# tnestmeyer/reflectance-filtering

Hardware: AMD Instinct MI355X
Metric: megapixels/sec joint-bilateral sigma_c=20 sigma_s=22 @1080p (higher is better)
Workload: dtype f32

## Files before the change

include/reflectance_filtering.h:

```cpp
#ifndef REFLECTANCE_FILTERING_H
#define REFLECTANCE_FILTERING_H

#include <stddef.h>
#include <stdint.h>

#ifdef __cplusplus
extern "C" {
#endif

#define RF_VERSION 103

#define RF_OK 0
#define RF_E_BADARG (-1)
#define RF_E_UNSUPPORTED (-2)
#define RF_E_WORKSPACE (-3)
#define RF_E_HIP (-4)

#define RF_BORDER_CONSTANT 0
#define RF_BORDER_REPLICATE 1
#define RF_BORDER_REFLECT 2
#define RF_BORDER_WRAP 3
#define RF_BORDER_REFLECT_101 4
#define RF_BORDER_DEFAULT RF_BORDER_REFLECT_101

#define RF_JBF_TRUE_DIVISION 1
#define RF_JBF_FORCE_GENERIC 2
#define RF_JBF_GREY_AS_BGR 4

int rf_version(void);
const char *rf_last_error(void);
int rf_shutdown(void);

int rf_jbf_u8(const uint8_t *joint, const uint8_t *src, uint8_t *dst, int n, int h, int w,
              int joint_cn, int src_cn, int d, double sigma_color, double sigma_space, int border,
              int flags, void *stream);

size_t rf_jbf_ragged_workspace_bytes(int n, const int *heights, const int *widths, int joint_cn,
                                     int src_cn, int d, double sigma_space, int flags);
int rf_jbf_ragged_u8(const uint8_t *joint, const uint8_t *src, uint8_t *dst, int n,
                     const int *heights, const int *widths, int joint_cn, int src_cn, int d,
                     double sigma_color, double sigma_space, int border, int flags, void *workspace,
                     size_t workspace_bytes, void *stream);

size_t rf_gf_workspace_bytes(int n, int h, int w, int guide_cn, int src_cn, int radius);
int rf_gf_u8(const uint8_t *guide, const uint8_t *src, uint8_t *dst, int n, int h, int w,
             int guide_cn, int src_cn, int radius, double eps, int iterations, void *workspace,
// ... 104 lines not shown
```

include/reflectance_filtering_debug.h:

```cpp
#ifndef REFLECTANCE_FILTERING_DEBUG_H
#define REFLECTANCE_FILTERING_DEBUG_H

#ifdef __cplusplus
extern "C" {
#endif

int rf_debug_option(const char *name, int value);

int rf_debug_clock_probe(unsigned long long *out2, int micros, void *stream);

const char *rf_debug_build_info(void);

int rf_debug_jbf_points_plan(int n_params, const double *sigma_space, int d, int joint_cn, int flags,
                             int total_points, int *out, int max_chunks);

int rf_debug_jbf_ragged_plan(int n, const int *heights, const int *widths, int joint_cn, int src_cn,
                             int d, double sigma_color, double sigma_space, int flags, int *out,
                             int cap);

int rf_debug_jbf_ragged_slab_plan(int n, const int *heights, const int *widths, int joint_cn,
                                  int src_cn, int d, double sigma_color, double sigma_space, int flags,
                                  int *out, int cap);

int rf_debug_colorize_ragged_plan(int n, const int *heights, const int *widths, int *out, int cap);

int rf_debug_gf_ragged_plan(int n, const int *heights, const int *widths, int guide_cn, int src_cn,
                            int radius, int flags, int *out, int cap);

int rf_debug_png_plan(int n, const int *heights, const int *widths, int cn_in, int flags, int *out,
                      int cap);

#ifdef __cplusplus
}
#endif
#endif
```

reflectance_filtering_amd/_ffi.py:

```python
import ctypes
import os
import threading

_HERE = os.path.dirname(os.path.abspath(__file__))
LIB_PATH = os.path.join(_HERE, "librf_hip.so")

RF_OK, RF_E_BADARG, RF_E_UNSUPPORTED, RF_E_WORKSPACE, RF_E_HIP = 0, -1, -2, -3, -4
BORDER_CONSTANT, BORDER_REPLICATE, BORDER_REFLECT, BORDER_WRAP, BORDER_REFLECT_101 = range(5)
BORDER_DEFAULT = BORDER_REFLECT_101
JBF_TRUE_DIVISION = 1
JBF_FORCE_GENERIC = 2
JBF_GREY_AS_BGR = 4
GF_GREY_AS_BGR = 1
PNG_GREY_AS_RGB = 1
PNG_FLAG_GREY, PNG_FLAG_BAD_FILTER = 1, 2
CNN_NPARAMS = 4513
CNN_NPACKED = 4673
CNN_NCHW_RGB, CNN_NHWC_BGR = 0, 1
CNN_LAYOUTS = {"nchw_rgb": CNN_NCHW_RGB, "nhwc_bgr": CNN_NHWC_BGR}

EXPORTS = ("rf_version", "rf_last_error", "rf_shutdown", "rf_jbf_u8", "rf_gf_workspace_bytes",
           "rf_gf_u8", "rf_gf_ex_u8", "rf_cnn_reflectance_u8", "rf_cnn_pack_weights",
           "rf_cnn_reflectance_packed_u8", "rf_colorize_workspace_bytes",
           "rf_colorize_srgb_u8", "rf_whdr_f32", "rf_jbf_f32_workspace_bytes", "rf_jbf_f32",
           "rf_gf_f32_workspace_bytes", "rf_gf_f32", "rf_jbf_points_workspace_bytes",
           "rf_jbf_points_u8", "rf_jbf_points_ragged_workspace_bytes", "rf_jbf_points_ragged_u8",
           "rf_whdr_points_u8", "rf_jbf_ragged_workspace_bytes", "rf_jbf_ragged_u8",
           "rf_colorize_ragged_workspace_bytes", "rf_colorize_ragged_srgb_u8",
           "rf_gf_ragged_workspace_bytes", "rf_gf_ragged_u8", "rf_png_stream_bound",
           "rf_png_workspace_bytes", "rf_png_deflate_ragged_u8",
           "rf_png_unfilter_workspace_bytes", "rf_png_unfilter_ragged_u8",
           "rf_colorize_ragged_r8_srgb_u8", "rf_cnn_reflectance_f32",
           "rf_cnn_reflectance_packed_f32")

DEBUG_EXPORTS = ("rf_debug_option", "rf_debug_clock_probe", "rf_debug_build_info",
                 "rf_debug_jbf_points_plan", "rf_debug_jbf_ragged_plan",
                 "rf_debug_jbf_ragged_slab_plan", "rf_debug_colorize_ragged_plan",
                 "rf_debug_gf_ragged_plan", "rf_debug_png_plan")
RESULT_CHANGING_OPTIONS = ("jbf_stage_only", "gf_exp_skip")

_lib = None
_lock = threading.Lock()


class RFError(RuntimeError):
    """A librf_hip.so entry point returned a negative code."""


def load_library():
    global _lib
    with _lock:
        if _lib is not None:
            return _lib
        import torch
        if not os.path.exists(LIB_PATH):
            raise RFError("%s not found: build it with `python -c 'import __graft_entry__ as g; "
                          "g.build()'` or `make -C reflectance_filtering_amd/csrc` "
                          "(there is no CPU fallback)" % LIB_PATH)
        lib = ctypes.CDLL(LIB_PATH)
        vp, ci, cd, sz = ctypes.c_void_p, ctypes.c_int, ctypes.c_double, ctypes.c_size_t
        lib.rf_version.argtypes = []
        lib.rf_version.restype = ci
        lib.rf_last_error.argtypes = []
        lib.rf_last_error.restype = ctypes.c_char_p
        lib.rf_shutdown.argtypes = []
        lib.rf_shutdown.restype = ci
        lib.rf_jbf_u8.argtypes = [vp, vp, vp, ci, ci, ci, ci, ci, ci, cd, cd, ci, ci, vp]
        lib.rf_jbf_u8.restype = ci
        lib.rf_gf_workspace_bytes.argtypes = [ci, ci, ci, ci, ci, ci]
        lib.rf_gf_workspace_bytes.restype = sz
        lib.rf_gf_u8.argtypes = [vp, vp, vp, ci, ci, ci, ci, ci, ci, cd, ci, vp, sz, vp]
        lib.rf_gf_u8.restype = ci
        lib.rf_gf_ex_u8.argtypes = [vp, vp, vp, ci, ci, ci, ci, ci, ci, cd, ci, ci, vp, sz, vp]
        lib.rf_gf_ex_u8.restype = ci
        lib.rf_gf_ragged_workspace_bytes.argtypes = [ci, vp, vp, ci, ci, ci, ci]
        lib.rf_gf_ragged_workspace_bytes.restype = sz
        lib.rf_gf_ragged_u8.argtypes = [vp, vp, vp, ci, vp, vp, ci, ci, ci, cd, ci, ci, vp, sz, vp]
        lib.rf_gf_ragged_u8.restype = ci
        lib.rf_cnn_reflectance_u8.argtypes = [vp, vp, vp, ci, ci, ci, vp, vp, vp]
        lib.rf_cnn_reflectance_u8.restype = ci
        lib.rf_cnn_pack_weights.argtypes = [vp, vp, vp]
# ... 55 lines not shown
        lib.rf_png_unfilter_ragged_u8.restype = ci
        lib.rf_debug_png_plan.argtypes = [ci, vp, vp, ci, ci, vp, ci]
        lib.rf_debug_png_plan.restype = ci
        lib.rf_debug_option.argtypes = [ctypes.c_char_p, ci]
        lib.rf_debug_option.restype = ci
        lib.rf_debug_clock_probe.argtypes = [vp, ci, vp]
        lib.rf_debug_clock_probe.restype = ci
        lib.rf_debug_build_info.argtypes = []
        lib.rf_debug_build_info.restype = ctypes.c_char_p
        lib.rf_debug_jbf_points_plan.argtypes = [ci, vp, ci, ci, ci, ci, vp, ci]
        lib.rf_debug_jbf_points_plan.restype = ci
        lib.rf_debug_jbf_ragged_plan.argtypes = [ci, vp, vp, ci, ci, ci, cd, cd, ci, vp, ci]
        lib.rf_debug_jbf_ragged_plan.restype = ci
        lib.rf_debug_jbf_ragged_slab_plan.argtypes = [ci, vp, vp, ci, ci, ci, cd, cd, ci, vp, ci]
        lib.rf_debug_jbf_ragged_slab_plan.restype = ci
        lib.rf_debug_colorize_ragged_plan.argtypes = [ci, vp, vp, vp, ci]
        lib.rf_debug_colorize_ragged_plan.restype = ci
        lib.rf_debug_gf_ragged_plan.argtypes = [ci, vp, vp, ci, ci, ci, ci, vp, ci]
        lib.rf_debug_gf_ragged_plan.restype = ci
        import sys
        for item in filter(None, os.environ.get("RF_DEBUG_OPTIONS", "").split(",")):
            name, _, value = item.partition("=")
            name = name.strip()
            try:
                number = int(value or 1)
            except ValueError:
                raise RFError("RF_DEBUG_OPTIONS: %r is not an integer (option %r)" % (value, name))
            if lib.rf_debug_option(name.encode(), number) < 0:
                raise RFError("RF_DEBUG_OPTIONS: unknown debug option %r" % name)
            if name in RESULT_CHANGING_OPTIONS and number:
# ... 82 lines not shown
    hs = np.ascontiguousarray(sizes[:, 0], dtype=np.int32)
    ws = np.ascontiguousarray(sizes[:, 1], dtype=np.int32)
    out = np.zeros(7, dtype=np.int32)
    args = (sizes.shape[0], hs.ctypes.data, ws.ctypes.data, int(joint_cn), int(src_cn), int(d),
            float(sigma_color), float(sigma_space), int(flags), out.ctypes.data, 1)
    rc = lib.rf_debug_jbf_ragged_slab_plan(*args)
    if rc == -1:
        if sizes.shape[0] == 0 or lib.rf_jbf_ragged_workspace_bytes(*(args[:6] + (args[7], args[8]))) > 0:
            return None
        lib.rf_debug_jbf_ragged_slab_plan(*args)
    if rc < 0:
        check(rc, "rf_debug_jbf_ragged_slab_plan")
    return tuple(int(v) for v in out)


def colorize_ragged_plan(sizes):
    import numpy as np
    lib = load_library()
    sizes = np.asarray(sizes, dtype=np.int64).reshape(-1, 2)
    n = sizes.shape[0]
    hs = np.ascontiguousarray(sizes[:, 0], dtype=np.int32)
    ws = np.ascontiguousarray(sizes[:, 1], dtype=np.int32)
    out = np.zeros(n + 2, dtype=np.int32)
    rc = lib.rf_debug_colorize_ragged_plan(n, hs.ctypes.data, ws.ctypes.data, out.ctypes.data, n + 2)
    if rc < 0:
        check(rc, "rf_debug_colorize_ragged_plan")
    return int(out[0]), int(out[1]), [int(v) for v in out[2:]]


def gf_ragged_plan(sizes, guide_cn, src_cn, radius, flags=0):
# ... 42 lines not shown
```

reflectance_filtering_amd/csrc/rf_api.hip:

```cpp
#include "rf_common.hpp"

#include <atomic>
#include <cstring>

#include "reflectance_filtering_debug.h"

namespace rf {

void jbf_shutdown();
void cnn_shutdown();
void gf_shutdown();

char *last_error_buf()
{
    static thread_local char buf[512] = "";
    return buf;
}

int fail(int code, const char *fmt, ...)
{
    va_list ap;
    va_start(ap, fmt);
    vsnprintf(last_error_buf(), 512, fmt, ap);
    va_end(ap);
// ... 6 lines not shown

}

extern "C" int rf_debug_option(const char *name, int value)
{
    static const char *const names[] = {"gf_two_kernel",     "jbf_stage_only",
                                                      "jbf_compiler_loop", "jbf_tile64_only",
                                                      "jbf_tune",          "jbf_f32_untiled",
                                                      "cnn_lds_columns",   "gf_seg_rows",
                                                      "gf_one_stream",     "gf_force_two_streams",
                                                      "gf_guide_cache",    "gf_chained",        "gf_no_compact",
                                                      "gf_exp_skip",       "gf_stagger",        "gf_parts",
                                                      "gf_s1_cap",         "gf_s1_min_wgs",
                                                      "jbf_lookahead1",    "gf_s1_legacy_strips",
                                                      "gf_exact_all_flagged", "gf_cw_chan_run",   "gf_exact",
                                                      "jbf_no_msad",       "colorize_chunk_px"};
    static_assert(sizeof(names) / sizeof(names[0]) == rf::kDbgCount, "one name per DebugOption");
    if (name)
        for (int i = 0; i < rf::kDbgCount; i++)
            if (std::strcmp(name, names[i]) == 0)
                return rf::g_debug[i].exchange(value < 0 ? 0 : value);
    return rf::fail(RF_E_BADARG, "rf_debug_option: unknown option '%s'", name ? name : "(null)");
}

__global__ void clock_probe_kernel(unsigned long long *out, unsigned long long ticks)
{
    if (threadIdx.x != 0)
        return;
    const unsigned long long r0 = __builtin_amdgcn_s_memrealtime();
    const unsigned long long c0 = __builtin_amdgcn_s_memtime();
    unsigned long long r1 = r0;
// ... 21 lines not shown
extern "C" int rf_version(void) { return RF_VERSION | 0x40000000; }
#else
extern "C" int rf_version(void) { return RF_VERSION; }
#endif

#ifndef RF_TOOLCHAIN
#define RF_TOOLCHAIN "unknown toolchain"
#endif
extern "C" const char *rf_debug_build_info(void) { return RF_TOOLCHAIN; }

extern "C" const char *rf_last_error(void) { return rf::last_error_buf(); }

extern "C" int rf_shutdown(void)
{
    rf::jbf_shutdown();
    rf::cnn_shutdown();
    rf::gf_shutdown();
    return RF_OK;
}
```

reflectance_filtering_amd/csrc/rf_common.hpp:

```cpp
#pragma once
#include <hip/hip_runtime.h>

#include <cstdarg>
#include <cstdint>
#include <cstdio>

#include "reflectance_filtering.h"

namespace rf {

char *last_error_buf();
int fail(int code, const char *fmt, ...);

#define RF_HIP_CHECK(expr)                                                                   \
    do {                                                                                     \
        hipError_t _e = (expr);                                                              \
        if (_e != hipSuccess)                                                                \
            return ::rf::fail(RF_E_HIP, "%s failed: %s (%s:%d)", #expr, hipGetErrorString(_e), \
                              __FILE__, __LINE__);                                           \
    } while (0)

__host__ __device__ inline int border_interpolate(int p, int len, int border)
{
    if ((unsigned)p < (unsigned)len)
// ... 60 lines not shown
    kDbgGfGuideCache,
    kDbgGfChained,
    kDbgGfNoCompact,
    kDbgGfExpSkip,
    kDbgGfStagger,
    kDbgGfParts,
    kDbgGfS1Cap,
    kDbgGfS1MinWgs,
    kDbgJbfLookahead1,
    kDbgGfS1LegacyStrips,
    kDbgGfExactAllFlagged,
    kDbgGfCwChanRun,
    kDbgGfExact,
    kDbgJbfNoMsad,
    kDbgColorizeChunkPx,
    kDbgCount
};
int debug_get(int id);

}
```

reflectance_filtering_amd/csrc/rf_jbf.hip:

```cpp
#include <algorithm>
#include <mutex>
#include <vector>

#include "rf_jbf_common.hpp"
#include "rf_jbf_tables.hpp"
#include "rf_jbf_taploops.hpp"

namespace rf {
namespace {

constexpr int kTileW = 64;
constexpr int kMaxLds = 160 * 1024;
constexpr int kTlw2 = 144;
constexpr int kJbfMaxTiledR4 = 468;
constexpr int kJbfStageOnly = 0x1000, kJbfCompilerLoop = 0x2000, kJbfTile64Only = 0x4000;
constexpr int kJbfLookahead1 = 0x8000;
constexpr int kJbfNoMsad = 0x10000;

int jbf_debug_flags()
{
    return (debug_get(kDbgJbfStageOnly) ? kJbfStageOnly : 0) |
           (debug_get(kDbgJbfCompilerLoop) ? kJbfCompilerLoop : 0) |
           (debug_get(kDbgJbfTile64Only) ? kJbfTile64Only : 0) |
           (debug_get(kDbgJbfLookahead1) ? kJbfLookahead1 : 0) |
           (debug_get(kDbgJbfNoMsad) ? kJbfNoMsad : 0);
}

__device__ inline void load_packed4(const uint8_t *img, size_t pix, int cn, uint32_t (&out)[4])
{
    const uint8_t *p = img + pix * (cn < 0 ? 1 : cn);
    if (cn == 3) {
        uint32_t d0, d1, d2;
// ... 242 lines not shown
struct alignas(16) JbfTileRec {
    unsigned long long first;
    int h, w, tile_y0, tile_x0, pad[2];
};
static_assert(sizeof(JbfTileRec) == 32, "the workspace holds 32 bytes per tile");

template <bool kRagged>
struct JbfTilesArg {
    using type = int;
};
template <>
struct JbfTilesArg<true> {
    using type = const JbfTileRec *__restrict__;
};

template <int SCN, int GREP, int CREP, int TLW, int TH = 64, bool kRagged = false>
__global__ __launch_bounds__(1024) void jbf_tile64_kernel(
    const uint8_t *__restrict__ joint, const uint8_t *__restrict__ src, uint8_t *__restrict__ dst,
    int h, int w, int jcn, int radius, int border, const float *__restrict__ lut, int nz,
    const int *__restrict__ hwtab, const float *__restrict__ swsym, int sw_len,
    typename JbfTilesArg<kRagged>::type tiles_x, int tiles_per_img, int flags, int crows, int y_base,
    int x_base)
{
    constexpr int NT = 1024;
    constexpr int QW = NT / TH;
    constexpr int TW = 4 * QW;
    static_assert(TH == 64 || TH == 32 || ((TH == 16 || TH == 128) && SCN == 1), "tile shapes");
    static_assert(QW >= 32 || (QW == 16 && TLW % 32 == 16) || (QW == 8 && TLW % 32 == 8),
                  "row pitch keeps the rows of a half-wave on disjoint banks");
    constexpr int Q4 = TLW / 4;
    extern __shared__ __align__(16) unsigned char smem[];
    volatile int *flag_word = reinterpret_cast<volatile int *>(smem);
    const bool need_sw = (flags & (kJbfCompilerLoop | kJbfLookahead1)) != 0;
    float *swl = reinterpret_cast<float *>(smem + 16);
    const int sw_bytes = need_sw ? ((radius + 1) * sw_len * 4 + 15) & ~15 : 0;
    unsigned char *tile_raw = smem + 16 + sw_bytes;
    if (threadIdx.x == 0)
        *flag_word = 3;
// ... 232 lines not shown
        w[i] = 0xdeadbeefu;
    __syncthreads();
    uint32_t bad = 0;
    const uint32_t addrs[4] = {(uint32_t)kT64Lds + 4u * threadIdx.x, (uint32_t)kT64Lds + 61056u,
                               262140u, (uint32_t)kT64Lds - 4u};
#pragma unroll
    for (int k = 0; k < 4; k++) {
        uint32_t v;
        asm volatile("ds_read_b32 %0, %1\n s_waitcnt lgkmcnt(0)" : "=v"(v) : "v"(addrs[k]));
        bad |= (k < 3) ? (v != 0u) : (v != 0xdeadbeefu);
    }
    if (bad)
        atomicOr(out, 1u);
}

struct Tiled2Config {
    int th, lutrep;
    bool full_lut;
};

size_t tiled2_lds_bytes(const JbfTables &t, int th, int lutrep, bool full_lut)
{
    const int lut_len = full_lut ? 256 * t.joint_cn : t.lut_len;
    const size_t lut_bytes = ((size_t)lut_len * lutrep * 4 + 15) & ~(size_t)15;
    const size_t sw_bytes = ((size_t)(t.radius + 1) * t.sw_len * 4 + 15) & ~(size_t)15;
    return 16 + lut_bytes + sw_bytes + (size_t)kTlw2 * (th + 2 * t.radius) * sizeof(uint2);
}

template <int SCN, int TH, int LUTREP>
int launch_tiled2(const JbfTables &t, bool full_lut, const uint8_t *joint, const uint8_t *src,
// ... 9 lines not shown
        return fail(RF_E_UNSUPPORTED, "rf_jbf_u8: batch too large for one launch");
    auto kern = clamp ? jbf_tiled2_kernel<SCN, TH, LUTREP, true>
                      : jbf_tiled2_kernel<SCN, TH, LUTREP, false>;
    RF_HIP_CHECK(hipFuncSetAttribute((const void *)kern, hipFuncAttributeMaxDynamicSharedMemorySize,
                                     (int)lds));
    hipLaunchKernelGGL(kern, dim3((unsigned)blocks), dim3(16 * TH), lds, stream, joint, src, dst, h,
                       w, jcn, t.radius, border, t.d_lut, lut_len, t.d_hw, t.d_swsym, t.sw_len,
                       tiles_x, tiles_x * tiles_y, flags);
    return RF_OK;
}


std::mutex g_oob_mu;
std::vector<int> g_oob_ok;

int lds_oob_reads_zero(int dev, bool *ok)
{
    {
        std::lock_guard<std::mutex> lock(g_oob_mu);
        if ((int)g_oob_ok.size() <= dev)
            g_oob_ok.resize(dev + 1, -1);
        if (g_oob_ok[dev] >= 0) {
            *ok = g_oob_ok[dev] == 1;
            return RF_OK;
        }
    }
    CaptureRelax relax;
    uint32_t *d_flag = nullptr;
    hipStream_t ps = nullptr;
    RF_HIP_CHECK(hipStreamCreateWithFlags(&ps, hipStreamNonBlocking));
    struct StreamGuard {
        hipStream_t s;
        ~StreamGuard() { (void)hipStreamDestroy(s); }
    } guard{ps};
    RF_HIP_CHECK(hipMalloc(&d_flag, sizeof(uint32_t)));
    RF_HIP_CHECK(hipMemsetAsync(d_flag, 0, sizeof(uint32_t), ps));
    RF_HIP_CHECK(hipFuncSetAttribute((const void *)lds_oob_probe_kernel,
                                     hipFuncAttributeMaxDynamicSharedMemorySize, kT64Lds));
    hipLaunchKernelGGL(lds_oob_probe_kernel, dim3(8), dim3(256), kT64Lds, ps, d_flag);
    uint32_t flag = 1;
    RF_HIP_CHECK(hipMemcpyAsync(&flag, d_flag, sizeof(flag), hipMemcpyDeviceToHost, ps));
    RF_HIP_CHECK(hipStreamSynchronize(ps));
    (void)hipFree(d_flag);
    std::lock_guard<std::mutex> lock(g_oob_mu);
    g_oob_ok[dev] = flag == 0 ? 1 : 0;
    *ok = flag == 0;
    return RF_OK;
}

int tile64_fits(const JbfTables &t, int nz, int grep, int crep, int scn, int tlw, int th, int flags)
{
    if (2 * t.r4 + 4 * (1024 / th) + 8 > tlw)
        return 0;
    const bool need_sw = (flags & (kJbfCompilerLoop | kJbfLookahead1)) != 0;
    const size_t sw_bytes =
        16 + (need_sw ? ((size_t)(t.radius + 1) * t.sw_len * 4 + 15) & ~(size_t)15 : 0);
    const size_t grey = sw_bytes + (size_t)tlw * (th + 2 * t.radius) * 4 + (size_t)nz * grep * 4;
    if (grey > (size_t)kT64Lds)
        return 0;
    if (scn == 1)
        return 32;
// ... 16 lines not shown
                  hipStream_t stream, int y_base = 0, int rows = -1, int x_base = 0, int cols = -1)
{
    if (rows < 0)
        rows = h;
    if (cols < 0)
        cols = w;
    const int tiles_x = ceil_div(cols, 4 * (1024 / TH)), tiles_y = ceil_div(rows, TH);
    const long long blocks = (long long)tiles_x * tiles_y * n;
    if (blocks > 0x7fffffffLL)
        return fail(RF_E_UNSUPPORTED, "rf_jbf_u8: batch too large for one launch");
    auto kern = jbf_tile64_kernel<SCN, GREP, CREP, TLW, TH>;
    RF_HIP_CHECK(hipFuncSetAttribute((const void *)kern, hipFuncAttributeMaxDynamicSharedMemorySize,
                                     kT64Lds));
    hipLaunchKernelGGL(kern, dim3((unsigned)blocks), dim3(1024), kT64Lds, stream, joint, src, dst,
                       h, w, jcn, t.radius, border, t.d_lut, nz, t.d_hw, t.d_swsym, t.sw_len,
                       tiles_x, tiles_x * tiles_y, flags, crows, y_base, x_base);
    return RF_OK;
}

struct Tile64Areas {
    int rows_main, cols_main, s32, s16, sx;
};

Tile64Areas tile64_areas(const JbfTables &t, int nz, int grep, int crep, int scn, int flags, int h,
                         int w)
{
    const bool only64 = (flags & kJbfTile64Only) != 0;
    int sx = 0;
    if (scn == 1 && !only64 && (w & 63) > 0 && (w & 63) <= 32 &&
        tile64_fits(t, nz, grep, crep, scn, 136, 128, flags) > 0 && ceil_div(h, 128) < ceil_div(h, 64))
        sx = w & 63;
// ... 6 lines not shown
        s16 = rem;
    else if (rem > 0 && rem <= 32 && ok32)
        s32 = rem;
    else if (rem > 32 && rem <= 48 && ok32 && ok16)
        s32 = 32, s16 = rem - 32;
    const int strip_blocks =
        (s32 ? ceil_div(cols_main, 128) : 0) + (s16 ? ceil_div(cols_main, 256) : 0);
    if (only64 || cols_main == 0 || ((s32 || s16) && strip_blocks >= ceil_div(cols_main, 64)))
        s32 = s16 = 0;
    return Tile64Areas{h - s32 - s16, cols_main, s32, s16, sx};
}

template <int SCN, int GREP, int CREP>
int launch_tile64_rows(const JbfTables &t, int nz, int crows, const uint8_t *joint,
                       const uint8_t *src, uint8_t *dst, int n, int h, int w, int jcn, int border,
                       int flags, hipStream_t stream)
{
    const Tile64Areas a = tile64_areas(t, nz, GREP, CREP, SCN, flags, h, w);
    const int rows_main = a.rows_main, cols_main = a.cols_main, s32 = a.s32, s16 = a.s16, sx = a.sx;
    int rc = RF_OK;
    if (rows_main > 0 && cols_main > 0)
        rc = launch_tile64<SCN, GREP, CREP, 144>(t, nz, crows, joint, src, dst, n, h, w, jcn,
                                                 border, flags, stream, 0, rows_main, 0, cols_main);
    if (rc == RF_OK && s32)
        rc = launch_tile64<SCN, GREP, CREP, 208, 32>(t, nz, 32, joint, src, dst, n, h, w, jcn,
                                                     border, flags, stream, rows_main, s32, 0,
                                                     cols_main);
    if constexpr (SCN == 1) {
        if (rc == RF_OK && s16)
            rc = launch_tile64<1, GREP, CREP, 336, 16>(t, nz, 32, joint, src, dst, n, h, w, jcn,
                                                       border, flags, stream, rows_main + s32, s16,
                                                       0, cols_main);
        if (rc == RF_OK && sx)
            rc = launch_tile64<1, GREP, CREP, 136, 128>(t, nz, 32, joint, src, dst, n, h, w, jcn,
                                                        border, flags, stream, 0, h, cols_main, sx);
    }
// ... 73 lines not shown

template <int SCN, int GREP, int CREP, int TLW, int TH>
int launch_tile64_ragged(const JbfTables &t, int nz, int crows, const uint8_t *joint,
                         const uint8_t *src, uint8_t *dst, const JbfTileRec *d_recs, size_t ntiles,
                         int jcn, int border, int flags, hipStream_t stream)
{
    if (ntiles == 0)
        return RF_OK;
    if (ntiles > (size_t)0x7fffffff)
        return fail(RF_E_UNSUPPORTED, "rf_jbf_ragged_u8: too many tiles for one launch");
    auto kern = jbf_tile64_kernel<SCN, GREP, CREP, TLW, TH, true>;
    RF_HIP_CHECK(hipFuncSetAttribute((const void *)kern, hipFuncAttributeMaxDynamicSharedMemorySize,
                                     kT64Lds));
    hipLaunchKernelGGL(kern, dim3((unsigned)ntiles), dim3(1024), kT64Lds, stream, joint, src, dst, 0,
                       0, jcn, t.radius, border, t.d_lut, nz, t.d_hw, t.d_swsym, t.sw_len, d_recs, 0,
                       flags, crows, 0, 0);
    return RF_OK;
}

template <int SCN, int GREP, int CREP, int TLW>
int launch_ragged(const JbfTables &t, int nz, const RaggedPlan &plan, const uint8_t *joint,
                  const uint8_t *src, uint8_t *dst, const JbfTileRec *const *d_recs, int jcn,
                  int border, int flags, hipStream_t stream)
{
    int rc = launch_tile64_ragged<SCN, GREP, CREP, TLW, 64>(t, nz, plan.shape.crows, joint, src, dst,
                                                            d_recs[0], plan.recs[0].size(), jcn,
                                                            border, flags, stream);
    if constexpr (TLW == 144) {
        if (rc == RF_OK)
            rc = launch_tile64_ragged<SCN, GREP, CREP, 208, 32>(t, nz, 32, joint, src, dst, d_recs[1],
                                                                plan.recs[1].size(), jcn, border,
// ... 208 lines not shown
                       int jcn, int scn, int border, int flags, hipStream_t stream)
{
    if (ntiles == 0)
        return RF_OK;
    if (ntiles > (size_t)0x7fffffff)
        return fail(RF_E_UNSUPPORTED, "rf_jbf_ragged_u8: too many tiles for one launch");
    auto kern = jbf_slab_kernel<GREP, TLW, true>;
    RF_HIP_CHECK(hipFuncSetAttribute((const void *)kern, hipFuncAttributeMaxDynamicSharedMemorySize,
                                     kT64Lds));
    hipLaunchKernelGGL(kern, dim3((unsigned)ntiles), dim3(1024), kT64Lds, stream, joint, src, dst, 0,
                       0, jcn, scn, t.radius, border, t.d_lut, nz, t.d_hw, t.d_swsym, t.sw_len,
                       d_recs, 0, flags, s.crows_g, s.slab_g, s.crows_c, s.slab_c);
    return RF_OK;
}

}
}

extern "C" int rf_jbf_u8(const uint8_t *joint, const uint8_t *src, uint8_t *dst, int n, int h,
                         int w, int joint_cn, int src_cn, int d, double sigma_color,
                         double sigma_space, int border, int flags, void *stream_)
{
    using namespace rf;
    if (n == 0)
        return RF_OK;
    if (!joint || !src || !dst)
        return fail(RF_E_BADARG, "rf_jbf_u8: NULL image pointer");
    if (n < 0 || h <= 0 || w <= 0)
        return fail(RF_E_BADARG, "rf_jbf_u8: bad size n=%d h=%d w=%d", n, h, w);
    if (int bad = jbf_check_format("rf_jbf_u8", joint_cn, src_cn, border))
        return bad;
// ... 14 lines not shown
    hipStream_t stream = (hipStream_t)stream_;
    const int jcn_kernel = jbf_kernel_cn(joint_cn, flags);
    joint_cn = jbf_table_cn(joint_cn, flags);
    JbfTables t;
    TablesHold hold{t};
    int rc = get_tables(radius, joint_cn, sigma_color, sigma_space, stream, &t);
    if (rc != RF_OK)
        return rc;

    const int tune = debug_get(kDbgJbfTune) & 0xf;
    static const Tiled2Config kCfg[] = {{48, 16, false}, {32, 8, true},  {32, 32, false},
                                        {32, 16, false}, {64, 16, false}, {48, 8, false}};
    constexpr int kNumCfg = (int)(sizeof(kCfg) / sizeof(kCfg[0]));
    bool done = false;
    if (!(flags & RF_JBF_FORCE_GENERIC) && t.r4 <= kJbfMaxTiledR4 && (tune == 0 || tune == 7)) {
        bool oob_ok = false;
        rc = lds_oob_reads_zero(t.device, &oob_ok);
        if (rc != RF_OK)
            return rc;
        const int nz = t.lut_len < 256 * joint_cn ? t.lut_len - 1 : t.lut_len;
        if (oob_ok) {
            Tile64Shape shape;
            if (tile64_choose(t, nz, src_cn, flags, &shape)) {
#define RF_T64(G_, C_, W_)                                                                        \
    if (shape.grep == G_ && shape.crep == C_ && shape.tlw == W_) {                                \
        if (W_ == 144)                                                                            \
            rc = src_cn == 3 ? launch_tile64_rows<3, G_, C_>(t, nz, shape.crows, joint, src, dst, \
                                                             n, h, w, jcn_kernel, border, flags,  \
                                                             stream)                              \
                             : launch_tile64_rows<1, G_, C_>(t, nz, shape.crows, joint, src, dst, \
                                                             n, h, w, jcn_kernel, border, flags,  \
                                                             stream);                             \
        else                                                                                      \
            rc = src_cn == 3 ? launch_tile64<3, G_, C_, W_>(t, nz, shape.crows, joint, src, dst,  \
                                                            n, h, w, jcn_kernel, border, flags,   \
                                                            stream)                               \
                             : launch_tile64<1, G_, C_, W_>(t, nz, shape.crows, joint, src, dst,  \
                                                            n, h, w, jcn_kernel, border, flags,   \
                                                            stream);                              \
    }
// ... 161 lines not shown
    std::vector<float> lut;
    const JbfTables t = jbf_host_tables(jbf_radius(d, jbf_sigma(sigma_space)),
                                        jbf_table_cn(joint_cn, flags), jbf_sigma(sigma_color),
                                        jbf_sigma(sigma_space), lut);
    RaggedPlan plan;
    plan_ragged(t, n, heights, widths, src_cn, flags | jbf_debug_flags(),
                debug_get(kDbgJbfTune) & 0xf, &plan);
    if (!plan.slab)
        return -1;
    if (cap > 0) {
        const SlabShape &s = plan.slab_shape;
        const int record[7] = {s.tlw, s.grep, s.crows_g, s.slab_g, s.crows_c, s.slab_c,
                               (int)std::min<size_t>(plan.recs[0].size(), 0x7fffffff)};
        std::copy(record, record + 7, out);
    }
    return 1;
}

extern "C" int rf_jbf_ragged_u8(const uint8_t *joint, const uint8_t *src, uint8_t *dst, int n,
                                const int *heights, const int *widths, int joint_cn, int src_cn,
                                int d, double sigma_color, double sigma_space, int border, int flags,
                                void *workspace, size_t workspace_bytes, void *stream_)
{
    using namespace rf;
    const char *who = "rf_jbf_ragged_u8";
    if (n == 0)
        return RF_OK;
    if (!joint || !src || !dst)
        return fail(RF_E_BADARG, "%s: NULL image pointer", who);
    size_t px, tiles;
// ... 92 lines not shown
```

reflectance_filtering_amd/ops.py:

```python
import numpy as np

from . import _ffi

_gf_workspaces = {}
_GF_CACHE_PER_DEVICE = 4
_GF_CACHE_BYTES_PER_DEVICE = 64 << 30
_cnn_consts = {}
_jbf_ragged_workspaces = {}
_colorize_ragged_workspaces = {}
_gf_ragged_workspaces = {}
_png_workspaces = {}
_png_decode_workspaces = {}


def release_workspaces():
    _png_workspaces.clear()
    _png_decode_workspaces.clear()
    del _png_host[:]
    _gf_workspaces.clear()
    _gf_ragged_workspaces.clear()
    _jbf_ragged_workspaces.clear()
    _colorize_ragged_workspaces.clear()
    _cnn_consts.clear()
    _steps_dev.clear()


def _chk_images(t, name, torch):
    if not (isinstance(t, torch.Tensor) and t.is_cuda and t.dtype == torch.uint8
            and t.dim() == 4 and t.is_contiguous()):
        raise ValueError("%s must be a contiguous CUDA uint8 tensor [N,H,W,C]" % name)
# ... 707 lines not shown
```

Measured before the change: 2415.

## Add two-workgroup-per-CU tile64 JBF path with per-tile grey voting

Adds a tile64x2 kernel that uses half the LDS (80 KB) and processes the vertical window in slabs, so two 1024-thread workgroups can share a CU. A vote pre-pass classifies each tile as grey or colour. Grey tiles go to the new single-channel kernel and colour tiles to the existing tile64 kernel, which is now gated by per-tile flags. This adds extra launches, a vote pass that rereads the halo, slab reloads and a new LDS out-of-bounds probe, in exchange for better occupancy and cheaper grey processing.

```diff
diff --git a/include/reflectance_filtering.h b/include/reflectance_filtering.h
--- a/include/reflectance_filtering.h
+++ b/include/reflectance_filtering.h
@@ -30,6 +30,7 @@
 int rf_version(void);
 const char *rf_last_error(void);
 int rf_shutdown(void);
+int rf_jbf_release_scratch(void);
 
 int rf_jbf_u8(const uint8_t *joint, const uint8_t *src, uint8_t *dst, int n, int h, int w,
               int joint_cn, int src_cn, int d, double sigma_color, double sigma_space, int border,
diff --git a/include/reflectance_filtering_debug.h b/include/reflectance_filtering_debug.h
--- a/include/reflectance_filtering_debug.h
+++ b/include/reflectance_filtering_debug.h
@@ -22,6 +22,11 @@
                                   int src_cn, int d, double sigma_color, double sigma_space, int flags,
                                   int *out, int cap);
 
+int rf_debug_jbf_two_wg_plan(int n, int h, int w, int joint_cn, int src_cn, int d, double sigma_color,
+                             double sigma_space, int flags, int *out);
+
+int rf_debug_jbf_two_wg_calls(void);
+
 int rf_debug_colorize_ragged_plan(int n, const int *heights, const int *widths, int *out, int cap);
 
 int rf_debug_gf_ragged_plan(int n, const int *heights, const int *widths, int guide_cn, int src_cn,
diff --git a/reflectance_filtering_amd/_ffi.py b/reflectance_filtering_amd/_ffi.py
--- a/reflectance_filtering_amd/_ffi.py
+++ b/reflectance_filtering_amd/_ffi.py
@@ -31,11 +31,13 @@
            "rf_png_workspace_bytes", "rf_png_deflate_ragged_u8",
            "rf_png_unfilter_workspace_bytes", "rf_png_unfilter_ragged_u8",
            "rf_colorize_ragged_r8_srgb_u8", "rf_cnn_reflectance_f32",
-           "rf_cnn_reflectance_packed_f32")
+           "rf_cnn_reflectance_packed_f32", "rf_jbf_release_scratch")
 
 DEBUG_EXPORTS = ("rf_debug_option", "rf_debug_clock_probe", "rf_debug_build_info",
                  "rf_debug_jbf_points_plan", "rf_debug_jbf_ragged_plan",
-                 "rf_debug_jbf_ragged_slab_plan", "rf_debug_colorize_ragged_plan",
+                 "rf_debug_jbf_ragged_slab_plan", "rf_debug_jbf_two_wg_plan",
+                 "rf_debug_jbf_two_wg_calls",
+                 "rf_debug_colorize_ragged_plan",
                  "rf_debug_gf_ragged_plan", "rf_debug_png_plan")
 RESULT_CHANGING_OPTIONS = ("jbf_stage_only", "gf_exp_skip")
 
@@ -65,6 +67,8 @@
         lib.rf_last_error.restype = ctypes.c_char_p
         lib.rf_shutdown.argtypes = []
         lib.rf_shutdown.restype = ci
+        lib.rf_jbf_release_scratch.argtypes = []
+        lib.rf_jbf_release_scratch.restype = ci
         lib.rf_jbf_u8.argtypes = [vp, vp, vp, ci, ci, ci, ci, ci, ci, cd, cd, ci, ci, vp]
         lib.rf_jbf_u8.restype = ci
         lib.rf_gf_workspace_bytes.argtypes = [ci, ci, ci, ci, ci, ci]
@@ -150,6 +154,10 @@
         lib.rf_debug_jbf_ragged_plan.restype = ci
         lib.rf_debug_jbf_ragged_slab_plan.argtypes = [ci, vp, vp, ci, ci, ci, cd, cd, ci, vp, ci]
         lib.rf_debug_jbf_ragged_slab_plan.restype = ci
+        lib.rf_debug_jbf_two_wg_plan.argtypes = [ci, ci, ci, ci, ci, ci, cd, cd, ci, vp]
+        lib.rf_debug_jbf_two_wg_plan.restype = ci
+        lib.rf_debug_jbf_two_wg_calls.argtypes = []
+        lib.rf_debug_jbf_two_wg_calls.restype = ci
         lib.rf_debug_colorize_ragged_plan.argtypes = [ci, vp, vp, vp, ci]
         lib.rf_debug_colorize_ragged_plan.restype = ci
         lib.rf_debug_gf_ragged_plan.argtypes = [ci, vp, vp, ci, ci, ci, ci, vp, ci]
@@ -262,6 +270,18 @@
     return tuple(int(v) for v in out)
 
 
+def jbf_two_wg_plan(n, h, w, joint_cn, src_cn, d, sigma_color, sigma_space, flags=0):
+    import numpy as np
+    lib = load_library()
+    out = np.zeros(4, dtype=np.int32)
+    rc = lib.rf_debug_jbf_two_wg_plan(int(n), int(h), int(w), int(joint_cn), int(src_cn), int(d),
+                                      float(sigma_color), float(sigma_space), int(flags),
+                                      out.ctypes.data)
+    if rc < 0:
+        check(rc, "rf_debug_jbf_two_wg_plan")
+    return tuple(int(v) for v in out[1:]) if rc == 1 else None
+
+
 def colorize_ragged_plan(sizes):
     import numpy as np
     lib = load_library()
diff --git a/reflectance_filtering_amd/csrc/rf_api.hip b/reflectance_filtering_amd/csrc/rf_api.hip
--- a/reflectance_filtering_amd/csrc/rf_api.hip
+++ b/reflectance_filtering_amd/csrc/rf_api.hip
@@ -8,6 +8,7 @@
 namespace rf {
 
 void jbf_shutdown();
+void jbf_scratch_release();
 void cnn_shutdown();
 void gf_shutdown();
 
@@ -44,7 +45,8 @@
                                                       "gf_s1_cap",         "gf_s1_min_wgs",
                                                       "jbf_lookahead1",    "gf_s1_legacy_strips",
                                                       "gf_exact_all_flagged", "gf_cw_chan_run",   "gf_exact",
-                                                      "jbf_no_msad",       "colorize_chunk_px"};
+                                                      "jbf_no_msad",       "colorize_chunk_px",
+                                                      "jbf_no_two_wg"};
     static_assert(sizeof(names) / sizeof(names[0]) == rf::kDbgCount, "one name per DebugOption");
     if (name)
         for (int i = 0; i < rf::kDbgCount; i++)
@@ -96,6 +98,7 @@
 extern "C" int rf_shutdown(void)
 {
     rf::jbf_shutdown();
+    rf::jbf_scratch_release();
     rf::cnn_shutdown();
     rf::gf_shutdown();
     return RF_OK;
diff --git a/reflectance_filtering_amd/csrc/rf_common.hpp b/reflectance_filtering_amd/csrc/rf_common.hpp
--- a/reflectance_filtering_amd/csrc/rf_common.hpp
+++ b/reflectance_filtering_amd/csrc/rf_common.hpp
@@ -98,6 +98,7 @@
     kDbgGfExact,
     kDbgJbfNoMsad,
     kDbgColorizeChunkPx,
+    kDbgJbfNoTwoWg,
     kDbgCount
 };
 int debug_get(int id);
diff --git a/reflectance_filtering_amd/csrc/rf_jbf.hip b/reflectance_filtering_amd/csrc/rf_jbf.hip
--- a/reflectance_filtering_amd/csrc/rf_jbf.hip
+++ b/reflectance_filtering_amd/csrc/rf_jbf.hip
@@ -1,4 +1,5 @@
 #include <algorithm>
+#include <atomic>
 #include <mutex>
 #include <vector>
 
@@ -16,6 +17,7 @@
 constexpr int kJbfStageOnly = 0x1000, kJbfCompilerLoop = 0x2000, kJbfTile64Only = 0x4000;
 constexpr int kJbfLookahead1 = 0x8000;
 constexpr int kJbfNoMsad = 0x10000;
+constexpr int kJbfVoteOnly = 0x20000;
 
 int jbf_debug_flags()
 {
@@ -288,14 +290,28 @@
     using type = const JbfTileRec *__restrict__;
 };
 
-template <int SCN, int GREP, int CREP, int TLW, int TH = 64, bool kRagged = false>
+struct JbfNoTileFlags {};
+template <bool kFlagged>
+struct JbfTileFlagsArg {
+    using type = JbfNoTileFlags;
+};
+template <>
+struct JbfTileFlagsArg<true> {
+    using type = const uint8_t *__restrict__;
+};
+
+template <int SCN, int GREP, int CREP, int TLW, int TH = 64, bool kRagged = false, bool kFlagged = false>
 __global__ __launch_bounds__(1024) void jbf_tile64_kernel(
     const uint8_t *__restrict__ joint, const uint8_t *__restrict__ src, uint8_t *__restrict__ dst,
     int h, int w, int jcn, int radius, int border, const float *__restrict__ lut, int nz,
     const int *__restrict__ hwtab, const float *__restrict__ swsym, int sw_len,
     typename JbfTilesArg<kRagged>::type tiles_x, int tiles_per_img, int flags, int crows, int y_base,
-    int x_base)
-{
+    int x_base, typename JbfTileFlagsArg<kFlagged>::type tile_flags)
+{
+    if constexpr (kFlagged) {
+        if ((tile_flags[xcd_contiguous_tile((int)blockIdx.x, (int)gridDim.x)] & 1) == 0)
+            return;
+    }
     constexpr int NT = 1024;
     constexpr int QW = NT / TH;
     constexpr int TW = 4 * QW;
@@ -558,6 +574,28 @@
         atomicOr(out, 1u);
 }
 
+constexpr int kT64x2Lds = 81920;
+
+__global__ __launch_bounds__(256) void lds_oob_probe_half_kernel(uint32_t *out)
+{
+    extern __shared__ __align__(16) unsigned char smem[];
+    uint32_t *w = reinterpret_cast<uint32_t *>(smem);
+    for (int i = threadIdx.x; i < kT64x2Lds / 4; i += blockDim.x)
+        w[i] = 0xdeadbeefu;
+    __syncthreads();
+    uint32_t bad = 0;
+    const uint32_t addrs[5] = {(uint32_t)kT64x2Lds + 4u * threadIdx.x, (uint32_t)kT64x2Lds + 61056u,
+                               (uint32_t)kT64Lds - 4u, 262140u, (uint32_t)kT64x2Lds - 4u};
+#pragma unroll
+    for (int k = 0; k < 5; k++) {
+        uint32_t v;
+        asm volatile("ds_read_b32 %0, %1\n s_waitcnt lgkmcnt(0)" : "=v"(v) : "v"(addrs[k]));
+        bad |= (k < 4) ? (v != 0u) : (v != 0xdeadbeefu);
+    }
+    if (bad)
+        atomicOr(out, 2u);
+}
+
 struct Tiled2Config {
     int th, lutrep;
     bool full_lut;
@@ -597,14 +635,16 @@
 std::mutex g_oob_mu;
 std::vector<int> g_oob_ok;
 
-int lds_oob_reads_zero(int dev, bool *ok)
+int lds_oob_reads_zero(int dev, bool *ok, bool *ok_half = nullptr)
 {
     {
         std::lock_guard<std::mutex> lock(g_oob_mu);
         if ((int)g_oob_ok.size() <= dev)
             g_oob_ok.resize(dev + 1, -1);
         if (g_oob_ok[dev] >= 0) {
-            *ok = g_oob_ok[dev] == 1;
+            *ok = (g_oob_ok[dev] & 1) != 0;
+            if (ok_half)
+                *ok_half = (g_oob_ok[dev] & 2) != 0;
             return RF_OK;
         }
     }
@@ -621,13 +661,18 @@
     RF_HIP_CHECK(hipFuncSetAttribute((const void *)lds_oob_probe_kernel,
                                      hipFuncAttributeMaxDynamicSharedMemorySize, kT64Lds));
     hipLaunchKernelGGL(lds_oob_probe_kernel, dim3(8), dim3(256), kT64Lds, ps, d_flag);
-    uint32_t flag = 1;
+    RF_HIP_CHECK(hipFuncSetAttribute((const void *)lds_oob_probe_half_kernel,
+                                     hipFuncAttributeMaxDynamicSharedMemorySize, kT64x2Lds));
+    hipLaunchKernelGGL(lds_oob_probe_half_kernel, dim3(2048), dim3(256), kT64x2Lds, ps, d_flag);
+    uint32_t flag = 3;
     RF_HIP_CHECK(hipMemcpyAsync(&flag, d_flag, sizeof(flag), hipMemcpyDeviceToHost, ps));
     RF_HIP_CHECK(hipStreamSynchronize(ps));
     (void)hipFree(d_flag);
     std::lock_guard<std::mutex> lock(g_oob_mu);
-    g_oob_ok[dev] = flag == 0 ? 1 : 0;
-    *ok = flag == 0;
+    g_oob_ok[dev] = (int)(~flag & 3u);
+    *ok = (flag & 1u) == 0;
+    if (ok_half)
+        *ok_half = (flag & 2u) == 0;
     return RF_OK;
 }
 
@@ -674,7 +719,7 @@
                                      kT64Lds));
     hipLaunchKernelGGL(kern, dim3((unsigned)blocks), dim3(1024), kT64Lds, stream, joint, src, dst,
                        h, w, jcn, t.radius, border, t.d_lut, nz, t.d_hw, t.d_swsym, t.sw_len,
-                       tiles_x, tiles_x * tiles_y, flags, crows, y_base, x_base);
+                       tiles_x, tiles_x * tiles_y, flags, crows, y_base, x_base, JbfNoTileFlags{});
     return RF_OK;
 }
 
@@ -711,12 +756,12 @@
 template <int SCN, int GREP, int CREP>
 int launch_tile64_rows(const JbfTables &t, int nz, int crows, const uint8_t *joint,
                        const uint8_t *src, uint8_t *dst, int n, int h, int w, int jcn, int border,
-                       int flags, hipStream_t stream)
+                       int flags, hipStream_t stream, bool strips_only = false)
 {
     const Tile64Areas a = tile64_areas(t, nz, GREP, CREP, SCN, flags, h, w);
     const int rows_main = a.rows_main, cols_main = a.cols_main, s32 = a.s32, s16 = a.s16, sx = a.sx;
     int rc = RF_OK;
-    if (rows_main > 0 && cols_main > 0)
+    if (rows_main > 0 && cols_main > 0 && !strips_only)
         rc = launch_tile64<SCN, GREP, CREP, 144>(t, nz, crows, joint, src, dst, n, h, w, jcn,
                                                  border, flags, stream, 0, rows_main, 0, cols_main);
     if (rc == RF_OK && s32)
@@ -820,7 +865,7 @@
                                      kT64Lds));
     hipLaunchKernelGGL(kern, dim3((unsigned)ntiles), dim3(1024), kT64Lds, stream, joint, src, dst, 0,
                        0, jcn, t.radius, border, t.d_lut, nz, t.d_hw, t.d_swsym, t.sw_len, d_recs, 0,
-                       flags, crows, 0, 0);
+                       flags, crows, 0, 0, JbfNoTileFlags{});
     return RF_OK;
 }
 
@@ -1059,7 +1104,289 @@
     return RF_OK;
 }
 
-}
+int tile64x2_slab_rows(int nz, int grep, int tlw)
+{
+    const int rows = (kT64x2Lds - nz * grep * 4) / (tlw * 4);
+    return rows >= 64 ? rows - 64 + 1 : 0;
+}
+
+template <int GREP, int TLW>
+__global__ __launch_bounds__(1024, 8) void jbf_tile64x2_kernel(
+    const uint8_t *__restrict__ joint, const uint8_t *__restrict__ src, uint8_t *__restrict__ dst,
+    int h, int w, int jcn, int scn, int radius, int border, const float *__restrict__ lut, int nz,
+    const int *__restrict__ hwtab, const float *__restrict__ swsym, int sw_len, int tiles_x,
+    int tiles_per_img, int flags, int slab_rows, uint8_t *__restrict__ tile_flags)
+{
+    constexpr int NT = 1024, Q4 = TLW / 4, QW = 16;
+    static_assert(TLW % 32 == 16, "row pitch keeps the rows of a half-wave on disjoint banks");
+    extern __shared__ __align__(16) unsigned char smem[];
+    int *flag_word = reinterpret_cast<int *>(smem);
+    uint32_t *tile4 = reinterpret_cast<uint32_t *>(smem);
+    const int tid = threadIdx.x;
+    if (tid == 0)
+        *flag_word = 3;
+    __syncthreads();
+    const int tile_id = xcd_contiguous_tile((int)blockIdx.x, (int)gridDim.x);
+    const int img_idx = tile_id / tiles_per_img;
+    const int t_in_img = tile_id - img_idx * tiles_per_img;
+    const int tile_y0 = (t_in_img / tiles_x) * 64;
+    const int tile_x0 = (t_in_img % tiles_x) * 64;
+    const size_t img = (size_t)img_idx * h * w;
+    const int r4 = (radius + 3) & ~3;
+    const int tx = tid % QW, ty = tid / QW;
+    int grey_joint = 1;
+    if (flags & kJbfVoteOnly) {
+        int grey = 1;
+        const int rows_all = 64 + 2 * radius;
+        for (int item = tid; item < rows_all * Q4; item += NT) {
+            const int ry = item / Q4, k = item - ry * Q4;
+            const int gy = border_interpolate(tile_y0 - radius + ry, h, border);
+            uint32_t jv[4], sv[4];
+            load_tile_quad(joint, src, img, gy, tile_x0 - r4 + 4 * k, w, jcn, scn, border, jv, sv);
+#pragma unroll
+            for (int u = 0; u < 4; u++) {
+                if (scn == 3)
+                    grey &= (int)(((sv[u] ^ (sv[u] >> 8)) & 0xffffu) == 0u);
+                if (jcn == 3)
+                    grey_joint &= (int)(((jv[u] ^ (jv[u] >> 8)) & 0xffffu) == 0u);
+            }
+        }
+        const int bits = block_all2(grey, grey_joint, flag_word);
+        if (tid == 0)
+            tile_flags[tile_id] = (uint8_t)(((bits & 1) ? 0 : 1) | (bits & 2));
+        return;
+    }
+    if (tile_flags) {
+        const int byte = __builtin_amdgcn_readfirstlane((int)tile_flags[tile_id]);
+        if (byte & 1)
+            return;
+        grey_joint = (byte >> 1) & 1;
+    }
+    float *lut_g = reinterpret_cast<float *>(smem + kT64x2Lds - nz * GREP * 4);
+    for (int i = tid; i < nz * GREP; i += NT)
+        lut_g[i] = lut[i / GREP];
+    const uint32_t lut_lane_addr = lds_addr(lut_g) + (uint32_t)(tid & (GREP - 1)) * 4u;
+    const uint32_t tile_lane_addr = lds_addr(tile4) + (uint32_t)tx * 4u;
+    const bool j1 = grey_joint != 0;
+    const uint32_t j1_scale = (uint32_t)(jcn == 1 ? 1 : 3) * (GREP * 4u);
+    uint32_t jc[kPix];
+    float sum1[kPix][1], wsum[kPix];
+    {
+        uint32_t jv[4], sv[4];
+        load_tile_quad(joint, src, img, border_interpolate(tile_y0 + ty, h, border), tile_x0 + 4 * tx, w, jcn,
+                       scn, border, jv, sv);
+#pragma unroll
+        for (int p = 0; p < kPix; p++) {
+            jc[p] = j1 ? (jv[p] & 0xffu) * j1_scale : jv[p] & 0x00ffffffu;
+            sum1[p][0] = 0.f;
+            wsum[p] = 0.f;
+        }
+    }
+    const bool msad = !j1 && !(flags & kJbfNoMsad) && jbf_wave_takes_msad(jc);
+    for (int i0 = -radius; i0 <= radius; i0 += slab_rows) {
+        const int i1 = min(i0 + slab_rows - 1, radius);
+        const int tlh = 64 + (i1 - i0);
+        __syncthreads();
+        for (int item = tid; item < tlh * Q4; item += NT) {
+            const int ry = item / Q4, k = item - ry * Q4;
+            const int gy = border_interpolate(tile_y0 + i0 + ry, h, border);
+            uint32_t jv[4], sv[4];
+            load_tile_quad(joint, src, img, gy, tile_x0 - r4 + 4 * k, w, jcn, scn, border, jv, sv);
+#pragma unroll
+            for (int u = 0; u < 4; u++) {
+                const uint32_t jfield = j1 ? (jv[u] & 0xffu) * j1_scale : jv[u];
+                tile4[ry * TLW + u * Q4 + k] = jfield | (sv[u] << 24);
+            }
+        }
+        __syncthreads();
+        if (j1)
+            jbf_tap_loop_grey4_la2<GREP, TLW, true, true>(lut_lane_addr, swsym, tile_lane_addr, jc, ty,
+                                                          radius, r4, sw_len, hwtab, sum1, wsum, i0, i1, -i0);
+        else if (msad)
+            jbf_tap_loop_grey4_la2<GREP, TLW, false, true, true>(lut_lane_addr, swsym, tile_lane_addr, jc,
+                                                                 ty, radius, r4, sw_len, hwtab, sum1, wsum,
+                                                                 i0, i1, -i0);
+        else
+            jbf_tap_loop_grey4_la2<GREP, TLW, false, true>(lut_lane_addr, swsym, tile_lane_addr, jc, ty,
+                                                           radius, r4, sw_len, hwtab, sum1, wsum, i0, i1,
+                                                           -i0);
+    }
+    if (scn == 1)
+        store_quad<1, 1>(dst, img, tile_y0 + ty, tile_x0 + 4 * tx, h, w, sum1, wsum, flags);
+    else
+        store_quad<1, 3>(dst, img, tile_y0 + ty, tile_x0 + 4 * tx, h, w, sum1, wsum, flags);
+}
+
+struct TileFlagBuf {
+    int dev;
+    hipStream_t stream;
+    uint8_t *p;
+    size_t bytes;
+};
+std::mutex g_tf_mu;
+std::vector<TileFlagBuf> g_tf;
+std::vector<uint8_t *> g_tf_retired;
+constexpr size_t kTileFlagStreams = 16;
+std::atomic<int> g_two_wg_calls{0};
+
+size_t tile_flag_bytes(size_t tiles)
+{
+    size_t b = 4096;
+    while (b < tiles)
+        b <<= 1;
+    return b;
+}
+
+int get_tile_flags(int dev, hipStream_t stream, size_t tiles, uint8_t **out)
+{
+    *out = nullptr;
+    std::lock_guard<std::mutex> lock(g_tf_mu);
+    size_t at = g_tf.size();
+    for (size_t i = 0; i < g_tf.size(); i++)
+        if (g_tf[i].dev == dev && g_tf[i].stream == stream)
+            at = i;
+    if (at < g_tf.size() && g_tf[at].bytes >= tiles) {
+        *out = g_tf[at].p;
+        return RF_OK;
+    }
+    hipStreamCaptureStatus st = hipStreamCaptureStatusNone;
+    if (hipStreamIsCapturing(stream, &st) != hipSuccess || st != hipStreamCaptureStatusNone) {
+        (void)hipGetLastError();
+        return RF_OK;
+    }
+    if (at == g_tf.size() && g_tf.size() >= kTileFlagStreams)
+        return RF_OK;
+    uint8_t *p = nullptr;
+    {
+        CaptureRelax relax;
+        RF_HIP_CHECK(hipMalloc(&p, tile_flag_bytes(tiles)));
+    }
+    if (at < g_tf.size()) {
+        g_tf_retired.push_back(g_tf[at].p);
+        g_tf.erase(g_tf.begin() + at);
+    }
+    g_tf.push_back(TileFlagBuf{dev, stream, p, tile_flag_bytes(tiles)});
+    *out = p;
+    return RF_OK;
+}
+
+bool two_wg_choose(const JbfTables &t, int nz, int src_cn, int flags, int *slab_rows)
+{
+    *slab_rows = 0;
+    if (debug_get(kDbgJbfNoTwoWg) || debug_get(kDbgJbfTune) ||
+        (flags & (RF_JBF_FORCE_GENERIC | kJbfStageOnly | kJbfCompilerLoop | kJbfLookahead1)))
+        return false;
+    Tile64Shape shape;
+    if (t.r4 > 36 || !tile64_choose(t, nz, src_cn, flags, &shape) || shape.tlw != 144 || shape.grep != 32)
+        return false;
+    *slab_rows = tile64x2_slab_rows(nz, 32, 144);
+    return *slab_rows >= 8;
+}
+
+int launch_tile64x2(const JbfTables &t, int nz, int slab_rows, const uint8_t *joint, const uint8_t *src,
+                    uint8_t *dst, int n, int h, int w, int jcn, int scn, int border, int flags,
+                    hipStream_t stream, int rows, int cols, uint8_t *tile_flags)
+{
+    const int tiles_x = ceil_div(cols, 64), tiles_y = ceil_div(rows, 64);
+    const long long blocks = (long long)tiles_x * tiles_y * n;
+    auto kern = jbf_tile64x2_kernel<32, 144>;
+    RF_HIP_CHECK(hipFuncSetAttribute((const void *)kern, hipFuncAttributeMaxDynamicSharedMemorySize,
+                                     kT64x2Lds));
+    hipLaunchKernelGGL(kern, dim3((unsigned)blocks), dim3(1024), kT64x2Lds, stream, joint, src, dst, h, w,
+                       jcn, scn, t.radius, border, t.d_lut, nz, t.d_hw, t.d_swsym, t.sw_len, tiles_x,
+                       tiles_x * tiles_y, flags, slab_rows, tile_flags);
+    return RF_OK;
+}
+
+template <int CREP>
+int launch_tile64_flagged(const JbfTables &t, int nz, int crows, const uint8_t *joint, const uint8_t *src,
+                          uint8_t *dst, int n, int h, int w, int jcn, int border, int flags,
+                          hipStream_t stream, int rows, int cols, const uint8_t *tile_flags)
+{
+    const int tiles_x = ceil_div(cols, 64), tiles_y = ceil_div(rows, 64);
+    const long long blocks = (long long)tiles_x * tiles_y * n;
+    auto kern = jbf_tile64_kernel<3, 32, CREP, 144, 64, false, true>;
+    RF_HIP_CHECK(hipFuncSetAttribute((const void *)kern, hipFuncAttributeMaxDynamicSharedMemorySize,
+                                     kT64Lds));
+    hipLaunchKernelGGL(kern, dim3((unsigned)blocks), dim3(1024), kT64Lds, stream, joint, src, dst, h, w,
+                       jcn, t.radius, border, t.d_lut, nz, t.d_hw, t.d_swsym, t.sw_len, tiles_x,
+                       tiles_x * tiles_y, flags, crows, 0, 0, tile_flags);
+    return RF_OK;
+}
+
+int launch_two_wg(const JbfTables &t, int nz, const Tile64Shape &shape, int slab_rows,
+                  const uint8_t *joint, const uint8_t *src, uint8_t *dst, int n, int h, int w, int jcn,
+                  int scn, int border, int flags, hipStream_t stream, bool *done)
+{
+    *done = false;
+    const Tile64Areas a = tile64_areas(t, nz, shape.grep, shape.crep, scn, flags, h, w);
+    if (a.rows_main <= 0 || a.cols_main <= 0)
+        return RF_OK;
+    const long long blocks = (long long)ceil_div(a.cols_main, 64) * ceil_div(a.rows_main, 64) * n;
+    if (blocks > 0x7fffffffLL)
+        return fail(RF_E_UNSUPPORTED, "rf_jbf_u8: batch too large for one launch");
+    uint8_t *tile_flags = nullptr;
+    int rc = RF_OK;
+    if (scn == 3 || jcn == 3) {
+        if (int bad = get_tile_flags(t.device, stream, (size_t)blocks, &tile_flags))
+            return bad;
+        if (!tile_flags)
+            return RF_OK;
+        rc = launch_tile64x2(t, nz, slab_rows, joint, src, dst, n, h, w, jcn, scn, border, flags | kJbfVoteOnly,
+                             stream, a.rows_main, a.cols_main, tile_flags);
+    }
+    if (rc == RF_OK && scn == 3)
+        rc = shape.crep == 32 ? launch_tile64_flagged<32>(t, nz, shape.crows, joint, src, dst, n, h, w, jcn,
+                                                          border, flags, stream, a.rows_main, a.cols_main,
+                                                          tile_flags)
+                              : launch_tile64_flagged<16>(t, nz, shape.crows, joint, src, dst, n, h, w, jcn,
+                                                          border, flags, stream, a.rows_main, a.cols_main,
+                                                          tile_flags);
+    if (rc == RF_OK)
+        rc = launch_tile64x2(t, nz, slab_rows, joint, src, dst, n, h, w, jcn, scn, border, flags, stream,
+                             a.rows_main, a.cols_main, tile_flags);
+    if (rc == RF_OK && (a.s32 || a.s16 || a.sx)) {
+        if (scn == 3)
+            rc = shape.crep == 32 ? launch_tile64_rows<3, 32, 32>(t, nz, shape.crows, joint, src, dst, n, h, w,
+                                                                  jcn, border, flags, stream, true)
+                                  : launch_tile64_rows<3, 32, 16>(t, nz, shape.crows, joint, src, dst, n, h, w,
+                                                                  jcn, border, flags, stream, true);
+        else
+            rc = shape.crep == 32 ? launch_tile64_rows<1, 32, 32>(t, nz, shape.crows, joint, src, dst, n, h, w,
+                                                                  jcn, border, flags, stream, true)
+                                  : launch_tile64_rows<1, 32, 16>(t, nz, shape.crows, joint, src, dst, n, h, w,
+                                                                  jcn, border, flags, stream, true);
+    }
+    *done = rc == RF_OK;
+    if (*done)
+        g_two_wg_calls.fetch_add(1, std::memory_order_relaxed);
+    return rc;
+}
+
+}
+
+void jbf_scratch_release()
+{
+    std::lock_guard<std::mutex> lock(g_tf_mu);
+    for (const TileFlagBuf &b : g_tf)
+        (void)hipFree(b.p);
+    for (uint8_t *p : g_tf_retired)
+        (void)hipFree(p);
+    g_tf.clear();
+    g_tf_retired.clear();
+}
+
+}
+
+extern "C" int rf_debug_jbf_two_wg_calls(void)
+{
+    return rf::g_two_wg_calls.load(std::memory_order_relaxed) & 0x7fffffff;
+}
+
+extern "C" int rf_jbf_release_scratch(void)
+{
+    rf::jbf_scratch_release();
+    return RF_OK;
 }
 
 extern "C" int rf_jbf_u8(const uint8_t *joint, const uint8_t *src, uint8_t *dst, int n, int h,
@@ -1104,16 +1431,23 @@
     constexpr int kNumCfg = (int)(sizeof(kCfg) / sizeof(kCfg[0]));
     bool done = false;
     if (!(flags & RF_JBF_FORCE_GENERIC) && t.r4 <= kJbfMaxTiledR4 && (tune == 0 || tune == 7)) {
-        bool oob_ok = false;
-        rc = lds_oob_reads_zero(t.device, &oob_ok);
+        bool oob_ok = false, oob_half = false;
+        rc = lds_oob_reads_zero(t.device, &oob_ok, &oob_half);
         if (rc != RF_OK)
             return rc;
         const int nz = t.lut_len < 256 * joint_cn ? t.lut_len - 1 : t.lut_len;
         if (oob_ok) {
             Tile64Shape shape;
             if (tile64_choose(t, nz, src_cn, flags, &shape)) {
+                int slab2 = 0;
+                if (oob_half && two_wg_choose(t, nz, src_cn, flags, &slab2)) {
+                    rc = launch_two_wg(t, nz, shape, slab2, joint, src, dst, n, h, w, jcn_kernel, src_cn,
+                                       border, flags, stream, &done);
+                    if (rc != RF_OK)
+                        return rc;
+                }
 #define RF_T64(G_, C_, W_)                                                                        \
-    if (shape.grep == G_ && shape.crep == C_ && shape.tlw == W_) {                                \
+    if (!done && shape.grep == G_ && shape.crep == C_ && shape.tlw == W_) {                       \
         if (W_ == 144)                                                                            \
             rc = src_cn == 3 ? launch_tile64_rows<3, G_, C_>(t, nz, shape.crows, joint, src, dst, \
                                                              n, h, w, jcn_kernel, border, flags,  \
@@ -1305,6 +1639,40 @@
                                (int)std::min<size_t>(plan.recs[0].size(), 0x7fffffff)};
         std::copy(record, record + 7, out);
     }
+    return 1;
+}
+
+extern "C" int rf_debug_jbf_two_wg_plan(int n, int h, int w, int joint_cn, int src_cn, int d,
+                                        double sigma_color, double sigma_space, int flags, int *out)
+{
+    using namespace rf;
+    const char *who = "rf_debug_jbf_two_wg_plan";
+    size_t px, tiles;
+    if (n < 1 || !out)
+        return fail(RF_E_BADARG, "%s: bad n=%d or NULL out", who, n);
+    if (int bad = ragged_check(who, 1, &h, &w, joint_cn, src_cn, d, sigma_space, RF_BORDER_DEFAULT, flags,
+                               &px, &tiles))
+        return bad;
+    std::vector<float> lut;
+    const JbfTables t = jbf_host_tables(jbf_radius(d, jbf_sigma(sigma_space)),
+                                        jbf_table_cn(joint_cn, flags), jbf_sigma(sigma_color),
+                                        jbf_sigma(sigma_space), lut);
+    flags |= jbf_debug_flags();
+    const int nz = t.lut_len < 256 * t.joint_cn ? t.lut_len - 1 : t.lut_len;
+    out[0] = out[1] = out[2] = out[3] = 0;
+    int slab_rows = 0;
+    Tile64Shape shape;
+    if (t.r4 > kJbfMaxTiledR4 || !two_wg_choose(t, nz, src_cn, flags, &slab_rows) ||
+        !tile64_choose(t, nz, src_cn, flags, &shape))
+        return 0;
+    const Tile64Areas a = tile64_areas(t, nz, shape.grep, shape.crep, src_cn, flags, h, w);
+    const long long blocks = (long long)ceil_div(a.cols_main, 64) * ceil_div(a.rows_main, 64) * n;
+    if (a.rows_main <= 0 || a.cols_main <= 0 || blocks > 0x7fffffffLL)
+        return 0;
+    out[0] = 1;
+    out[1] = 64 + slab_rows - 1;
+    out[2] = (int)blocks;
+    out[3] = src_cn == 3 || joint_cn == 3 ? (int)tile_flag_bytes((size_t)blocks) : 0;
     return 1;
 }
 
diff --git a/reflectance_filtering_amd/ops.py b/reflectance_filtering_amd/ops.py
--- a/reflectance_filtering_amd/ops.py
+++ b/reflectance_filtering_amd/ops.py
@@ -14,6 +14,8 @@
 
 
 def release_workspaces():
+    if _ffi._lib is not None:
+        _ffi._lib.rf_jbf_release_scratch()
     _png_workspaces.clear()
     _png_decode_workspaces.clear()
     del _png_host[:]
```

Measured after the change: 2617, median of 6. 8.3% higher.
